# zhengyk19/vit-rpe-rope

Hardware: AMD Instinct MI355X
Metric: train images/sec, CIFAR-10 ViT d=192 L=6 H=6 (higher is better)
Workload: dtype bf16; 1 GPU; CIFAR-10-shaped 32x32 patch4 ViT d=192 L=6 H=6, --pos_encoding rope-axial theta=100, bf16, full train step (fwd+CE+bwd+AdamW), random-init weights; per_gpu_batch=512, global_batch=512, parallelism=dp1, hip_graph=True

## Files before the change

### include/vitpe_debug.h

```cpp
#ifndef VITPE_DEBUG_H
#define VITPE_DEBUG_H
#include "vitpe.h"
#ifdef __cplusplus
extern "C" {
#endif

int vitpe_selftest_mma(int dtype, const void* A, const void* Bt, const void* Brow, float* C_row,
                       float* C_tr, vitpe_stream_t stream);

int vitpe_debug_wgrad_census(int dtype, const vitpe_wgrad_problem* problems, int nprob, unsigned long long* census,
                             vitpe_stream_t stream);
int vitpe_debug_attn_census(const void* xn, const void* wqkv, void* out, const float* cos, const float* sin,
                            int B, unsigned long long* census, vitpe_stream_t stream);
int vitpe_debug_attn32_census(const void* xn, const void* wqkv_wide, void* out, const float* cos, const float* sin,
                              int B, unsigned long long* census, vitpe_stream_t stream);
int vitpe_debug_tail2_census(const void* attn_out, const void* x_in, const void* Wp_packed, const float* bp,
                             const float* gamma, const float* beta, void* x_mid, float* mean2, float* rstd2,
                             void* xn_out, const void* W1_packed, const float* b1, const void* W2_packed,
                             const float* b2, void* gp_out, void* h_out, void* out, float* mean_out, float* rstd_out,
                             int M, int HID, unsigned long long* census, vitpe_stream_t stream);
int vitpe_debug_set_gemm2d_mt(int mt);
int vitpe_debug_set_wgrad_wide(int on);
int vitpe_debug_read_bw(const void* src, long long bytes, int depth, int workgroups, unsigned* sink, vitpe_stream_t stream);
#ifdef __cplusplus
}
#endif
#endif
```

### vit-rpe-rope_amd/csrc/attn.hip

```cpp
#include "attn_common.h"
#include <stdlib.h>
#include <type_traits>

namespace vitpe {

template <typename T, typename C, int KM, int NTH = 384>
VITPE_DEV void stage_tokens(const AttnArgs& a, int b, T* xs, T* hbuf, int hbuf_elems, float* s_tab, float* s_coef,
                            int tid, int nthreads, bool stage_tables) {
  constexpr int CHN = CH<T>::n;
  constexpr int DCH = C::LDX / CHN;
  constexpr int D = C::DD;
  const int N = C::ntok(a);
  const T* xg = reinterpret_cast<const T*>(a.xn) + (size_t)b * N * D;
  const Chunk16 zero = {0u, 0u, 0u, 0u};
  constexpr int TOTAL = C::NP * DCH;
  constexpr int ITERS = (TOTAL + NTH - 1) / NTH;
  Chunk16 v[ITERS];
#pragma unroll
  for (int it = 0; it < ITERS; ++it) {
    const int q = tid + it * nthreads, row = q / DCH, cc = q % DCH;
    v[it] = zero;
    if (q < TOTAL && row < N && cc * CHN < D) v[it] = *reinterpret_cast<const Chunk16*>(xg + (size_t)row * D + cc * CHN);
  }
  if (a.ln_gamma != nullptr) {
// ... 378 lines not shown
VITPE_DEV void stage_rows_plain(const T* src, T* dst, int ld, int N, int tid) {
  constexpr int CHN = CH<T>::n, D = C::DD, CPRW = D / CHN, RPP = NTH / CPRW, ITERS = C::NP / RPP;
  const int cc = tid % CPRW, r0 = tid / CPRW;
  const Chunk16 zero = {0u, 0u, 0u, 0u};
  Chunk16 v[ITERS];
#pragma unroll
  for (int it = 0; it < ITERS; ++it) {
    const int row = r0 + it * RPP;
    v[it] = *reinterpret_cast<const Chunk16*>(src + (size_t)min(row, N - 1) * D + cc * CHN);
    if (row >= N) v[it] = zero;
  }
#pragma unroll
  for (int it = 0; it < ITERS; ++it) *reinterpret_cast<Chunk16*>(dst + (r0 + it * RPP) * ld + cc * CHN) = v[it];
}

template <int HD, int D, int MT, int KM, int NTOK, int IPW, bool LNF, bool MIXED, int PDEG = 7>
__global__ __launch_bounds__(64 * (D / HD) * IPW, 3) void attn_bwd_reg_kernel(AttnArgs a) {
  using T = bf16;
  using C = AttnCfg<T, HD, D, MT, 1, NTOK>;
  constexpr int NT = C::NT, KS = C::KS, HC = C::HC, SC = C::SC, NTH = 64 * C::H;
  static_assert(NT == 2 && HC == 1, "head dimension 32");
  constexpr int CSLD = HD / 2 + 8;
  constexpr int FRAG = 64 * 8;
  constexpr int XS_ELEMS = IPW * C::NP * C::LDX, DOS_ELEMS = IPW * C::H * MT * FRAG;
  __shared__ __attribute__((aligned(16))) T xs_all[XS_ELEMS > DOS_ELEMS ? XS_ELEMS : DOS_ELEMS];
  __shared__ __attribute__((aligned(16))) T qs_all[IPW * C::H * MT * FRAG];
  __shared__ __attribute__((aligned(16))) float s_tab[KM == KM_RELATIVE ? C::H * C::TABLD : 4];
  __shared__ __attribute__((aligned(16))) float s_coef[KM == KM_POLY ? C::PESZ : 4];
  __shared__ __attribute__((aligned(16))) float s_cos[KM == KM_ROPE ? C::NP * CSLD : 4];
  __shared__ __attribute__((aligned(16))) float s_sin[KM == KM_ROPE ? C::NP * CSLD : 4];
  __shared__ __attribute__((aligned(16))) float s_stat[IPW * C::H * 2 * C::NP];
  __shared__ float s_dtab[KM == KM_RELATIVE ? C::H * C::TABLD : 4];
  __shared__ float s_dcoef[C::H * (C::MAXDEG + 1)];
  __shared__ float s_dfreq[2 * C::H * (HD / 2)];

  const int N = C::ntok(a), P = N - 1;
  const int lane = threadIdx.x & 63;
  const int wave_all = __builtin_amdgcn_readfirstlane(threadIdx.x >> 6);
  const int img = wave_all / C::H, h = wave_all % C::H;
  const int b_raw = blockIdx.x * IPW + img;
  const bool live = b_raw < a.B;
  const int b = live ? b_raw : a.B - 1;
  const int tid_img = threadIdx.x % NTH;
  T* const xs = xs_all + img * C::NP * C::LDX;
  T* const qsw = qs_all + wave_all * MT * FRAG + lane * 8;
  T* const dsw = xs_all + wave_all * MT * FRAG + lane * 8;
  float* const lse_w = s_stat + (img * C::H + h) * 2 * C::NP;
  float* const del_w = lse_w + C::NP;
  float* const dtab_i = s_dtab;
  float* const dcoef_i = s_dcoef;
  float* const dfreq_i = s_dfreq;
  const int c = lane & 15, g = lane >> 4;
  const f32x4 z4 = {0.f, 0.f, 0.f, 0.f};
  constexpr bool mixed = (KM == KM_ROPE) && MIXED;

  const T* const Wh = reinterpret_cast<const T*>(a.wqkv) + ((size_t)h * 3 * NT * KS * 64 + lane) * 8;
  auto wload = [&](Frag<T> (&w)[NT][KS], int mat) {
#pragma unroll
    for (int nt = 0; nt < NT; ++nt)
#pragma unroll
      for (int ks = 0; ks < KS; ++ks) w[nt][ks] = ld_frag(Wh + (size_t)((mat * NT + nt) * KS + ks) * 64 * 8);
  };
  Frag<T> w[NT][KS];
  wload(w, 2);
  stage_tokens_fwd<T, C, KM, NTH, LNF>(a, b, xs, s_tab, s_coef, tid_img, false, IPW == 1 || img == 0);
  if (KM == KM_ROPE && !mixed) {
    constexpr int F4 = HD / 8;
    for (int q = threadIdx.x; q < C::NP * F4; q += NTH * IPW) {
      const int f4 = q % F4, row = q / F4;
      f32x4 cv = {1.f, 1.f, 1.f, 1.f}, sv = {0.f, 0.f, 0.f, 0.f};
      if (row >= 1 && row < N) {
        cv = *reinterpret_cast<const f32x4*>(a.cos + (size_t)(row - 1) * (HD / 2) + 4 * f4);
        sv = *reinterpret_cast<const f32x4*>(a.sin + (size_t)(row - 1) * (HD / 2) + 4 * f4);
      }
      *reinterpret_cast<f32x4*>(&s_cos[row * CSLD + 4 * f4]) = cv;
      *reinterpret_cast<f32x4*>(&s_sin[row * CSLD + 4 * f4]) = sv;
    }
  }
  if (KM == KM_RELATIVE)
    for (int q = threadIdx.x; q < C::H * C::TABLD; q += NTH * IPW) s_dtab[q] = 0.f;
  for (int q = threadIdx.x; q < C::H * (C::MAXDEG + 1); q += NTH * IPW) s_dcoef[q] = 0.f;
  for (int q = threadIdx.x; q < 2 * C::H * (HD / 2); q += NTH * IPW) s_dfreq[q] = 0.f;
  __syncthreads();

  const T* const xrow = xs + c * C::LDX + 8 * g;
  const unsigned hoff = mixed ? (unsigned)(h * P * (HD / 2)) : 0u;
  auto cs_vec = [&](int tok, int f, f32x4& cv, f32x4& sv) {
    if (!mixed) {
      cv = *reinterpret_cast<const f32x4*>(&s_cos[tok * CSLD + f]);
      sv = *reinterpret_cast<const f32x4*>(&s_sin[tok * CSLD + f]);
    } else {
      const bool ok = tok >= 1 && tok < N;
      const unsigned o = hoff + (unsigned)((min(max(tok, 1), N - 1) - 1) * (HD / 2) + f);
      const f32x4 cg = *reinterpret_cast<const f32x4*>(a.cos + o), sg = *reinterpret_cast<const f32x4*>(a.sin + o);
      cv = ok ? cg : (f32x4){1.f, 1.f, 1.f, 1.f};
      sv = ok ? sg : z4;
    }
  };
  auto proj_sw = [&](int tt, bool rope, float sc, Frag<T>& dst) {
    Frag<T> xf[KS];
#pragma unroll
    for (int ks = 0; ks < KS; ++ks) xf[ks] = ld_frag(xrow + 16 * tt * C::LDX + 32 * ks);
    __builtin_amdgcn_sched_barrier(0);
    f32x4 acc[NT] = {z4, z4};
#pragma unroll
    for (int ks = 0; ks < KS; ++ks)
#pragma unroll
      for (int nt = 0; nt < NT; ++nt) mma(w[nt][ks], xf[ks], acc[nt]);
    __builtin_amdgcn_sched_barrier(0);
    if (KM == KM_ROPE && rope) {
      f32x4 cv, sv;
      cs_vec(16 * tt + c, 4 * g, cv, sv);
      const f32x4 x1 = acc[0], x2 = acc[1];
      acc[0] = x1 * cv - x2 * sv;
      acc[1] = x1 * sv + x2 * cv;
    }
    dst = acc_to_frag<T>(acc[0] * sc, acc[1] * sc);
    asm volatile("" : "+v"(dst.v));
  };
  Frag<T> e0, e1;
#pragma unroll
  for (int t = 0; t < 8; ++t) {
    e0.v[t] = (bf16)((t < 4 && 4 * g + t == c) ? 1.0f : 0.0f);
    e1.v[t] = (bf16)((t >= 4 && 4 * g + t - 4 == c) ? 1.0f : 0.0f);
  }
  auto transpose_pair = [&](const Frag<T>& fa, const Frag<T>* fb, Frag<T>& d0, Frag<T>& d1) {
    f32x4 a0 = z4, a1 = z4, b0 = z4, b1 = z4;
    mma(fa, e0, a0);
    mma(fa, e1, a1);
    if (fb != nullptr) { mma(*fb, e0, b0); mma(*fb, e1, b1); }
    d0 = acc_to_frag<T>(a0, b0);
    d1 = acc_to_frag<T>(a1, b1);
  };

  const float qsc = a.scale * LOG2E;
  Frag<T> vkf[MT], kf[MT];
#pragma unroll
  for (int tt = 0; tt < MT; ++tt) proj_sw(tt, false, 1.0f, vkf[tt]);
  wload(w, 1);
  __builtin_amdgcn_sched_barrier(0);
#pragma unroll
  for (int tt = 0; tt < MT; ++tt) proj_sw(tt, true, 1.0f, kf[tt]);
  wload(w, 0);
  __builtin_amdgcn_sched_barrier(0);
#pragma unroll
  for (int tt = 0; tt < MT; ++tt) {
    Frag<T> qf;
    proj_sw(tt, true, qsc, qf);
    *reinterpret_cast<bf16x8*>(qsw + tt * FRAG) = qf.v;
  }
  __syncthreads();
  if (!live) return;
  {
    const T* dog = reinterpret_cast<const T*>(a.dout) + (size_t)b * N * D + h * HD;
    Frag<T> df[MT];
#pragma unroll
    for (int tt = 0; tt < MT; ++tt) {
      const int tok = 16 * tt + c;
      bf16x4 lo = {(bf16)0.f, (bf16)0.f, (bf16)0.f, (bf16)0.f}, hi = lo;
      if (tok < N) {
        lo = *reinterpret_cast<const bf16x4*>(dog + (size_t)tok * D + 4 * g);
        hi = *reinterpret_cast<const bf16x4*>(dog + (size_t)tok * D + 16 + 4 * g);
      }
      df[tt].v = __builtin_shufflevector(lo, hi, 0, 1, 2, 3, 4, 5, 6, 7);
    }
#pragma unroll
    for (int tt = 0; tt < MT; ++tt) *reinterpret_cast<bf16x8*>(dsw + tt * FRAG) = df[tt].v;
  }
  auto qf_load = [&](int tt) { Frag<T> f; f.v = *reinterpret_cast<const bf16x8*>(qsw + tt * FRAG); return f; };
  auto dof_load = [&](int tt) { Frag<T> f; f.v = *reinterpret_cast<const bf16x8*>(dsw + tt * FRAG); return f; };
  Frag<T> ktf[NT][SC];
#pragma unroll
  for (int scx = 0; scx < SC; ++scx)
    transpose_pair(kf[2 * scx], (2 * scx + 1 < MT) ? &kf[(2 * scx + 1 < MT) ? 2 * scx + 1 : 0] : nullptr, ktf[0][scx], ktf[1][scx]);

  T* const dqg = reinterpret_cast<T*>(a.out) + (size_t)b * N * 3 * D + h * HD;
  auto store_pair = [&](T* rowp, const f32x4& o0, const f32x4& o1, bool ok) {
    uint32_t lo[2], hi[2];
#pragma unroll
    for (int w2 = 0; w2 < 2; ++w2) {
      bf16x2 pa, pb;
      pa[0] = (bf16)o0[2 * w2]; pa[1] = (bf16)o0[2 * w2 + 1];
      pb[0] = (bf16)o1[2 * w2]; pb[1] = (bf16)o1[2 * w2 + 1];
      const auto r = __builtin_amdgcn_permlane16_swap(__builtin_bit_cast(uint32_t, pa), __builtin_bit_cast(uint32_t, pb), false, false);
      lo[w2] = r[0]; hi[w2] = r[1];
    }
    const int f0 = 16 * (g & 1) + 8 * (g >> 1);
    if (ok) *reinterpret_cast<Chunk16*>(rowp + f0) = (Chunk16){lo[0], lo[1], hi[0], hi[1]};
  };

  float cacc[PDEG + 1];
#pragma unroll
  for (int k = 0; k <= PDEG; ++k) cacc[k] = 0.f;
#pragma unroll
  for (int it = 0; it < MT; ++it) {
    __builtin_amdgcn_sched_barrier(0);
    const int i = 16 * it + c;
    const Frag<T> dof = dof_load(it), qfi = qf_load(it);
    f32x4 s[MT], dp[MT];
    float m = -1e30f;
    typedef __attribute__((ext_vector_type(4))) unsigned u32x4;
    const unsigned xyi = (KM == KM_POLY) ? reinterpret_cast<const unsigned*>(s_coef + C::H * C::PBLD)[i] : 0u;
    const float* const ptab = s_coef + (a.coeff_per_head ? h : 0) * C::PBLD;
    const bool qcls = (it == 0) && (c == 0);
#pragma unroll
    for (int jt = 0; jt < MT; ++jt) {
      s[jt] = z4;
      mma(kf[jt], qfi, s[jt]);
      dp[jt] = z4;
      mma(vkf[jt], dof, dp[jt]);
      const u32x4 xyj = (KM == KM_POLY) ? *reinterpret_cast<const u32x4*>(s_coef + C::H * C::PBLD + 16 * jt + 4 * g) : (u32x4){0u, 0u, 0u, 0u};
#pragma unroll
      for (int r = 0; r < 4; ++r) {
        const int j = 16 * jt + 4 * g + r;
        float v = s[jt][r];
        if (KM == KM_RELATIVE) v += pe_bias2<C, KM>(a, s_tab, s_coef, h, i, j, N);
        if (KM == KM_POLY) {
          const float bv = ptab[__builtin_amdgcn_sad_u8(xyi, xyj[r], 0u)];
          const bool cls = qcls || (jt == 0 && r == 0 && g == 0);
          v += cls ? 0.f : bv;
        }
        if (jt == MT - 1) v = (j < N) ? v : -1e30f;
        s[jt][r] = v;
        m = fmaxf(m, v);
      }
    }
    m = xg_max(m);
    float l = 0.f;
#pragma unroll
    for (int jt = 0; jt < MT; ++jt)
#pragma unroll
      for (int r = 0; r < 4; ++r) { const float p = __builtin_amdgcn_exp2f(s[jt][r] - m); s[jt][r] = p; l += p; }
    l = xg_sum(l);
    const float inv = __builtin_amdgcn_rcpf(l);
    float dl = 0.f;
#pragma unroll
    for (int jt = 0; jt < MT; ++jt)
#pragma unroll
      for (int r = 0; r < 4; ++r) { s[jt][r] *= inv; dl += s[jt][r] * dp[jt][r]; }
    dl = xg_sum(dl);
    if (g == 0) { lse_w[i] = m + __builtin_amdgcn_logf(l); del_w[i] = dl; }
    const bool qvalid = (it < MT - 1) || (i < N);
    float tacc[PDEG + 1];
#pragma unroll
    for (int k = 0; k <= PDEG; ++k) tacc[k] = 0.f;
#pragma unroll
    for (int jt = 0; jt < MT; ++jt) {
      if (KM == KM_POLY) __builtin_amdgcn_sched_barrier(0);
      const u32x4 xyj = (KM == KM_POLY) ? *reinterpret_cast<const u32x4*>(s_coef + C::H * C::PBLD + 16 * jt + 4 * g) : (u32x4){0u, 0u, 0u, 0u};
#pragma unroll
// ... 5 lines not shown
        if (KM == KM_POLY) {
          const float dsk = (jt == 0 && r == 0) ? (g == 0 ? 0.f : ds) : ds;
          const float x = (float)__builtin_amdgcn_sad_u8(xyi, xyj[r], 0u);
          float pw = x;
          tacc[0] += dsk;
#pragma unroll
          for (int k = 1; k <= PDEG; ++k) { tacc[k] = fmaf(dsk, pw, tacc[k]); if (k < PDEG) pw *= x; }
        }
      }
    }
    if (KM == KM_POLY) {
      const float qm = (it == 0 && c == 0) ? 0.f : 1.f;
#pragma unroll
      for (int k = 0; k <= PDEG; ++k) {
        cacc[k] = fmaf(qm, tacc[k], cacc[k]);
        asm volatile("" : "+v"(cacc[k]));
      }
    }
    if (KM == KM_RELATIVE) {
#pragma unroll
      for (int jt = 0; jt < MT; ++jt) {
        float d0, d1;
        tile_diag_sums(dp[jt], lane, d0, d1);
        const int idx0 = 16 * (it - jt) + c + N - 1;
        if (g == 0) {
          if (idx0 >= 0 && idx0 <= 2 * N - 2) atomicAdd(&dtab_i[h * C::TABLD + idx0], d0);
          if (c >= 1 && idx0 - 16 >= 0 && idx0 - 16 <= 2 * N - 2) atomicAdd(&dtab_i[h * C::TABLD + idx0 - 16], d1);
        }
      }
    }
    f32x4 dqa[NT] = {z4, z4};
#pragma unroll
    for (int scx = 0; scx < SC; ++scx) {
      const Frag<T> bs = acc_to_frag<T>(dp[2 * scx], (2 * scx + 1 < MT) ? dp[(2 * scx + 1 < MT) ? 2 * scx + 1 : 0] : z4);
#pragma unroll
      for (int dt = 0; dt < NT; ++dt) mma(ktf[dt][scx], bs, dqa[dt]);
    }
    if (mixed) {
      const bool tok_ok = i >= 1 && i < N;
      f32x4 dph;
#pragma unroll
      for (int r = 0; r < 4; ++r) dph[r] = dqa[1][r] * (float)qfi.v[r] - dqa[0][r] * (float)qfi.v[4 + r];
      mixed_freq_grad_tile(dfreq_i, dph, i, tok_ok, 16 * it, h, C::H, P, a.grid, HD / 2, 4 * g, LN2, lane);
    }
    if (KM == KM_ROPE) {
      f32x4 cv, sv;
      cs_vec(min(i, C::NP - 1), 4 * g, cv, sv);
      const f32x4 d1 = dqa[0], d2 = dqa[1];
      dqa[0] = d1 * cv + d2 * sv;
      dqa[1] = d2 * cv - d1 * sv;
    }
    store_pair(dqg + (size_t)i * 3 * D, dqa[0] * a.scale, dqa[1] * a.scale, qvalid);
  }

  if (KM == KM_POLY) {
#pragma unroll
    for (int k = 0; k <= PDEG; ++k)
      if (k <= a.degree) {
        const float t = wave_sum(cacc[k]);
        if (lane == 0) atomicAdd(&dcoef_i[(a.coeff_per_head ? h : 0) * (C::MAXDEG + 1) + k], t);
      }
  }
  Frag<T> qtf[NT][SC], dotf[NT][SC];
  __builtin_amdgcn_sched_barrier(0);
#pragma unroll
  for (int scx = 0; scx < SC; ++scx) {
    const bool two = 2 * scx + 1 < MT;
    const Frag<T> qa = qf_load(2 * scx), qb = qf_load(two ? 2 * scx + 1 : 0);
    transpose_pair(qa, two ? &qb : nullptr, qtf[0][scx], qtf[1][scx]);
    const Frag<T> da = dof_load(2 * scx), db = dof_load(two ? 2 * scx + 1 : 0);
    transpose_pair(da, two ? &db : nullptr, dotf[0][scx], dotf[1][scx]);
  }
  __builtin_amdgcn_s_waitcnt(0xC07F);

#pragma unroll
  for (int jt = 0; jt < MT; ++jt) {
    __builtin_amdgcn_sched_barrier(0);
    const int j = 16 * jt + c;
    const bool kvalid = (jt < MT - 1) || (j < N);
    const unsigned xyk = (KM == KM_POLY) ? reinterpret_cast<const unsigned*>(s_coef + C::H * C::PBLD)[j] : 0u;
    const float* const ptab2 = s_coef + (a.coeff_per_head ? h : 0) * C::PBLD;
    const bool kcls = (jt == 0) && (c == 0);
    f32x4 p[MT], ds[MT];
#pragma unroll
    for (int it = 0; it < MT; ++it) {
      const Frag<T> dof = dof_load(it), qfi = qf_load(it);
      p[it] = z4;
      mma(qfi, kf[jt], p[it]);
      ds[it] = z4;
      mma(dof, vkf[jt], ds[it]);
      const f32x4 lse = *reinterpret_cast<const f32x4*>(&lse_w[16 * it + 4 * g]);
      const f32x4 dlv = *reinterpret_cast<const f32x4*>(&del_w[16 * it + 4 * g]);
      typedef __attribute__((ext_vector_type(4))) unsigned u32x4;
      const u32x4 xyq = (KM == KM_POLY) ? *reinterpret_cast<const u32x4*>(s_coef + C::H * C::PBLD + 16 * it + 4 * g) : (u32x4){0u, 0u, 0u, 0u};
#pragma unroll
      for (int r = 0; r < 4; ++r) {
        const int i = 16 * it + 4 * g + r;
        float sv = p[it][r];
        if (KM == KM_RELATIVE) sv += pe_bias2<C, KM>(a, s_tab, s_coef, h, i, j, N);
        if (KM == KM_POLY) {
          const float bv = ptab2[__builtin_amdgcn_sad_u8(xyk, xyq[r], 0u)];
          const bool cls = kcls || (it == 0 && r == 0 && g == 0);
          sv += cls ? 0.f : bv;
        }
        const bool valid = kvalid && ((it < MT - 1) || (i < N));
        const float pv = valid ? __builtin_amdgcn_exp2f(sv - lse[r]) : 0.f;
        p[it][r] = pv;
        ds[it][r] = pv * (ds[it][r] - dlv[r]);
      }
    }
    f32x4 dva[NT] = {z4, z4}, dka[NT] = {z4, z4};
#pragma unroll
    for (int scx = 0; scx < SC; ++scx) {
      const bool two = (2 * scx + 1 < MT);
      const Frag<T> bp = acc_to_frag<T>(p[2 * scx], two ? p[two ? 2 * scx + 1 : 0] : z4);
      const Frag<T> bs = acc_to_frag<T>(ds[2 * scx], two ? ds[two ? 2 * scx + 1 : 0] : z4);
#pragma unroll
      for (int dt = 0; dt < NT; ++dt) {
        mma(dotf[dt][scx], bp, dva[dt]);
        mma(qtf[dt][scx], bs, dka[dt]);
      }
    }
    dka[0] *= LN2; dka[1] *= LN2;
    if (mixed) {
      const bool tok_ok = j >= 1 && j < N;
      f32x4 dph;
#pragma unroll
      for (int r = 0; r < 4; ++r) dph[r] = dka[1][r] * (float)kf[jt].v[r] - dka[0][r] * (float)kf[jt].v[4 + r];
      mixed_freq_grad_tile(dfreq_i, dph, j, tok_ok, 16 * jt, h, C::H, P, a.grid, HD / 2, 4 * g, 1.0f, lane);
    }
    if (KM == KM_ROPE) {
      f32x4 cv, sv;
      cs_vec(min(j, C::NP - 1), 4 * g, cv, sv);
      const f32x4 d1 = dka[0], d2 = dka[1];
      dka[0] = d1 * cv + d2 * sv;
      dka[1] = d2 * cv - d1 * sv;
    }
    store_pair(dqg + (size_t)j * 3 * D + D, dka[0], dka[1], kvalid);
    store_pair(dqg + (size_t)j * 3 * D + 2 * D, dva[0], dva[1], kvalid);
  }

  __syncthreads();
  const int nrun = NTH * min(IPW, a.B - (int)blockIdx.x * IPW);
  if (KM == KM_RELATIVE) {
    for (int q = threadIdx.x; q < C::H * (2 * N - 1); q += nrun) {
      const int hh = q / (2 * N - 1), i = q % (2 * N - 1);
      atomicAdd(a.dtable + q, s_dtab[hh * C::TABLD + i]);
    }
  } else if (KM == KM_POLY) {
    const int nh = a.coeff_per_head ? C::H : 1;
    for (int q = threadIdx.x; q < nh * (a.degree + 1); q += nrun) {
      const int hh = q / (a.degree + 1), k = q % (a.degree + 1);
      atomicAdd(a.dcoeff + q, s_dcoef[hh * (C::MAXDEG + 1) + k]);
    }
  } else if (mixed) {
    for (int q = threadIdx.x; q < 2 * C::H * (HD / 2); q += nrun) atomicAdd(a.dfreqs + q, s_dfreq[q]);
  }
}

template <typename T, int HD, int D, int MT, int HPP, int KM, int NTOK>
__global__ __launch_bounds__(384) void attn_bwd_kernel(AttnArgs a) {
  using C = AttnCfg<T, HD, D, MT, HPP, NTOK>;
  __shared__ __attribute__((aligned(16))) T xs[C::NP * C::LDX];
  __shared__ __attribute__((aligned(16))) T hb[4 * HPP * C::HSZ];
  __shared__ __attribute__((aligned(16))) float s_tab[KM == KM_RELATIVE ? C::H * C::TABLD : 4];
  __shared__ __attribute__((aligned(16))) float s_coef[KM == KM_POLY ? C::PESZ : 4];
  __shared__ __attribute__((aligned(16))) float s_stat[HPP * 2 * C::NP];
  __shared__ float s_dtab[KM == KM_RELATIVE ? C::H * C::TABLD : 4];
  __shared__ float s_dcoef[C::H * (C::MAXDEG + 1)];
  __shared__ float s_dfreq[2 * C::H * (HD / 2)];
  constexpr int SLD = HPP * HD + Pad<T>::elems;
  __shared__ __attribute__((aligned(16))) T s_dq[3 * C::NP * SLD];

  const int N = C::ntok(a);
  const int b = blockIdx.x;
  const int lane = threadIdx.x & 63;
  const int wave = __builtin_amdgcn_readfirstlane(threadIdx.x >> 6);
  const int c = lane & 15, g = lane >> 4;
  const int P = N - 1;
  WFrags<T, C> wf;
  {
    const int hh = wave / 3, mat = wave % 3;
    if (hh < HPP && hh < C::H) load_w<T, C>(a, wf, hh, mat, lane);
  }
  stage_tokens<T, C, KM>(a, b, xs, hb, 4 * HPP * C::HSZ, s_tab, s_coef, threadIdx.x, 384, true);
  if (KM == KM_RELATIVE)
    for (int q = threadIdx.x; q < C::H * C::TABLD; q += 384) s_dtab[q] = 0.f;
  for (int q = threadIdx.x; q < C::H * (C::MAXDEG + 1); q += 384) s_dcoef[q] = 0.f;
  for (int q = threadIdx.x; q < 2 * C::H * (HD / 2); q += 384) s_dfreq[q] = 0.f;
  __syncthreads();

  constexpr int CHN = CH<T>::n;
  const T* dog = reinterpret_cast<const T*>(a.dout) + (size_t)b * N * D;
// ... 340 lines not shown
    if (a.ln_gamma != nullptr) hipLaunchKernelGGL((attn_fwd_kernel<T, HD, D, MT, KM, NTOK, IPW, true>), grid, block, 0, s, a);
    else hipLaunchKernelGGL((attn_fwd_kernel<T, HD, D, MT, KM, NTOK, IPW, false>), grid, block, 0, s, a);
  }
  VITPE_CHECK_LAUNCH();
}

template <typename T, int HD, int D, int MT, int HPP, int NTOK>
static int launch_attn2(bool bwd, const AttnArgs& a, hipStream_t s) {
  switch (a.mode) {
    case PE_RELATIVE: return launch_attn3<T, HD, D, MT, HPP, KM_RELATIVE, NTOK>(bwd, a, s);
    case PE_POLY: return launch_attn3<T, HD, D, MT, HPP, KM_POLY, NTOK>(bwd, a, s);
    case PE_ROPE_AXIAL:
    case PE_ROPE_MIXED: return launch_attn3<T, HD, D, MT, HPP, KM_ROPE, NTOK>(bwd, a, s);
    default: return launch_attn3<T, HD, D, MT, HPP, KM_PLAIN, NTOK>(bwd, a, s);
  }
}

template <typename T, int HD, int D, int MT, int HPP>
static int launch_attn(bool bwd, const AttnArgs& a, hipStream_t s) {
  if (a.N == 65) return launch_attn2<T, HD, D, MT, HPP, 65>(bwd, a, s);
  return launch_attn2<T, HD, D, MT, HPP, 0>(bwd, a, s);
}

static int dispatch_attn(bool bwd, int dtype, int D, int HD, const AttnArgs& a, hipStream_t s) {
  const int MT = (a.N + 15) / 16;
  if (HD != 32 || MT != 5) return (int)hipErrorNotSupported;
  if (dtype == 1) {
    if (D == 192) return launch_attn<bf16, 32, 192, 5, 2>(bwd, a, s);
    if (D == 96) return launch_attn<bf16, 32, 96, 5, 2>(bwd, a, s);
  } else if (dtype == 0) {
    if (D == 192) return launch_attn<float, 32, 192, 5, 1>(bwd, a, s);
    if (D == 96) return launch_attn<float, 32, 96, 5, 1>(bwd, a, s);
  }
  return (int)hipErrorNotSupported;
}

extern "C" int vitpe_fused_attention_supported(int dtype, int N, int D, int HD) {
  const int MT = (N + 15) / 16;
  return (dtype == 0 || dtype == 1) && HD == 32 && MT == 5 && (D == 192 || D == 96);
}

static int fused_fwd(int dtype, const void* x, const float* gamma, const float* beta, const float* mean,
                     const float* rstd, void* xn_out, const void* wqkv, void* out, int B, int N, int D, int HD,
                     const PeArgs& pe, hipStream_t stream) {
  VITPE_REQUIRE(x && wqkv && out && B >= 0 && N >= 2);
  VITPE_REQUIRE(pe_ok(pe, N, 0, 0));
  if (B == 0) return 0;
  AttnArgs a = attn_args(pe, B, N, 0, HD);
  a.xn = x; a.wqkv = wqkv; a.out = out;
  a.ln_gamma = gamma; a.ln_beta = beta; a.ln_mean = mean; a.ln_rstd = rstd; a.xn_out = xn_out;
  return dispatch_attn(false, dtype, D, HD, a, stream);
}

static int fused_bwd(int dtype, const void* x, const float* gamma, const float* beta, const float* mean,
                     const float* rstd, const void* wqkv, const void* dout, void* dqkv, int B, int N, int D, int HD,
                     const PeArgs& pe, float* dtable, float* dcoeff, float* dfreqs, hipStream_t stream) {
  VITPE_REQUIRE(x && wqkv && dout && dqkv && B >= 0 && N >= 2);
  VITPE_REQUIRE(pe_ok(pe, N, 0, 0));
  VITPE_REQUIRE(pe_grads_ok(pe.mode, dtable, dcoeff, dfreqs));
  if (B == 0) return 0;
  AttnArgs a = attn_args(pe, B, N, 0, HD);
  a.xn = x; a.wqkv = wqkv; a.out = dqkv; a.dout = dout;
  a.dtable = dtable; a.dcoeff = dcoeff; a.dfreqs = dfreqs;
  a.ln_gamma = gamma; a.ln_beta = beta; a.ln_mean = mean; a.ln_rstd = rstd;
  return dispatch_attn(true, dtype, D, HD, a, stream);
}

extern "C" int vitpe_fused_attention_fwd(int dtype, const void* xn, const void* wqkv, void* out, int B, int N,
                                         int D, int HD, int mode, const float* cos, const float* sin,
                                         const float* table, const float* coeff, int grid, int degree,
                                         int coeff_per_head, hipStream_t stream) {
  return fused_fwd(dtype, xn, nullptr, nullptr, nullptr, nullptr, nullptr, wqkv, out, B, N, D, HD,
                   {mode, cos, sin, table, coeff, grid, degree, coeff_per_head}, stream);
}

extern "C" int vitpe_fused_attention_fwd_ln(int dtype, const void* x, const float* gamma, const float* beta,
                                            const float* mean, const float* rstd, void* xn_out, const void* wqkv,
                                            void* out, int B, int N, int D, int HD, int mode, const float* cos,
                                            const float* sin, const float* table, const float* coeff, int grid,
                                            int degree, int coeff_per_head, hipStream_t stream) {
  VITPE_REQUIRE(gamma && beta && mean && rstd);
  return fused_fwd(dtype, x, gamma, beta, mean, rstd, xn_out, wqkv, out, B, N, D, HD,
                   {mode, cos, sin, table, coeff, grid, degree, coeff_per_head}, stream);
}

extern "C" int vitpe_fused_attention_bwd(int dtype, const void* xn, const void* wqkv, const void* dout,
                                         void* dqkv, int B, int N, int D, int HD, int mode, const float* cos,
                                         const float* sin, const float* table, const float* coeff, int grid,
                                         int degree, int coeff_per_head, float* dtable, float* dcoeff,
                                         float* dfreqs, hipStream_t stream) {
  return fused_bwd(dtype, xn, nullptr, nullptr, nullptr, nullptr, wqkv, dout, dqkv, B, N, D, HD,
                   {mode, cos, sin, table, coeff, grid, degree, coeff_per_head}, dtable, dcoeff, dfreqs, stream);
}

extern "C" int vitpe_fused_attention_bwd_ln(int dtype, const void* x, const float* gamma, const float* beta,
                                            const float* mean, const float* rstd, const void* wqkv, const void* dout,
                                            void* dqkv, int B, int N, int D, int HD, int mode, const float* cos,
                                            const float* sin, const float* table, const float* coeff, int grid,
                                            int degree, int coeff_per_head, float* dtable, float* dcoeff,
                                            float* dfreqs, hipStream_t stream) {
  VITPE_REQUIRE(gamma && beta && mean && rstd);
  return fused_bwd(dtype, x, gamma, beta, mean, rstd, wqkv, dout, dqkv, B, N, D, HD,
                   {mode, cos, sin, table, coeff, grid, degree, coeff_per_head}, dtable, dcoeff, dfreqs, stream);
}

extern "C" int vitpe_debug_attn_census(const void* xn, const void* wqkv, void* out, const float* cos, const float* sin,
                                       int B, unsigned long long* census, hipStream_t stream) {
  VITPE_REQUIRE(xn && wqkv && out && cos && sin && census && B > 0);
  AttnArgs a = attn_args({PE_ROPE_AXIAL, cos, sin, nullptr, nullptr, 8, 0, 0}, B, 65, 0, 32);
  a.xn = xn; a.wqkv = wqkv; a.out = out; a.census = census;
  hipLaunchKernelGGL((attn_fwd_kernel<bf16, 32, 192, 5, KM_ROPE, 65, 2, false, true>), dim3((B + 1) / 2), dim3(768), 0, stream, a);
  VITPE_CHECK_LAUNCH();
}
```

### vit-rpe-rope_amd/csrc/attn_common.h

```cpp
#pragma once
#include "common.h"

namespace vitpe {

struct AttnArgs {
  const void* xn;
  const void* wqkv;
  void* out;
  const void* dout;
  const float* cos;
  const float* sin;
  const float* table;
  const float* coeff;
  float* dtable;
  float* dcoeff;
  float* dfreqs;
  const void* qkv;
  int B, N, H;
  int mode, grid, degree, coeff_per_head;
  float scale;
  const float* ln_gamma;
  const float* ln_beta;
  const float* ln_mean;
  const float* ln_rstd;
  void* xn_out;
  unsigned long long* census;
  void* qkv_out;
  float* tab_slab;
  const unsigned long long* rng;
  unsigned drop_thr;
  float drop_rs;
  int cls_only;
};

struct PeArgs {
  int mode;
  const float *cos, *sin, *table, *coeff;
  int grid, degree, coeff_per_head;
};

inline bool pe_ok(const PeArgs& pe, int N, int H, int hmax) {
  if (pe.mode == PE_ROPE_AXIAL || pe.mode == PE_ROPE_MIXED) {
    if (!pe.cos || !pe.sin || pe.grid * pe.grid != N - 1) return false;
    if (pe.mode == PE_ROPE_MIXED && hmax && H > hmax) return false;
  }
  if (pe.mode == PE_RELATIVE && !pe.table) return false;
  if (pe.mode == PE_POLY && (!pe.coeff || pe.degree < 0 || pe.degree > 7 || pe.grid * pe.grid != N - 1)) return false;
  return pe.mode >= PE_NONE && pe.mode <= PE_ROPE_MIXED;
}

inline bool pe_grads_ok(int mode, const float* dtable, const float* dcoeff, const float* dfreqs) {
  if (mode == PE_RELATIVE) return dtable != nullptr;
  if (mode == PE_POLY) return dcoeff != nullptr;
  if (mode == PE_ROPE_MIXED) return dfreqs != nullptr;
  return true;
}

inline AttnArgs attn_args(const PeArgs& pe, int B, int N, int H, int HD) {
  AttnArgs a{};
  a.cos = pe.cos; a.sin = pe.sin; a.table = pe.table; a.coeff = pe.coeff;
  a.mode = pe.mode; a.grid = pe.grid; a.degree = pe.degree; a.coeff_per_head = pe.coeff_per_head;
  a.B = B; a.N = N; a.H = H;
  a.scale = 1.0f / sqrtf((float)HD);
  return a;
}

constexpr float LOG2E = 1.4426950408889634f;
constexpr float LN2 = 0.6931471805599453f;

enum { KM_PLAIN = 0, KM_RELATIVE = 1, KM_POLY = 2, KM_ROPE = 3, KM_ROPE_TABLES = 4 };

template <typename T, int HD, int D, int MT, int HPP, int NTOK>
struct AttnCfg {
  static constexpr int H = D / HD;
  static constexpr int NT = HD / 16;
  static constexpr int KS = D / 32;
  static constexpr int HC = HD / 32;
  static constexpr int NP = 16 * MT;
  static constexpr int SC = (MT + 1) / 2;
  static constexpr int VR = 32 * SC;
  static constexpr int LDX = D + (sizeof(T) == 2 ? 2 : 1) * Pad<T>::elems;
  static constexpr int LDH = HD + (sizeof(T) == 2 ? 2 : 1) * Pad<T>::elems;
  static constexpr int HSZ = VR * LDH;
  static constexpr int QSZ = NP * LDH;
  static constexpr int TABLD = 2 * NP;
// ... 133 lines not shown
```

### vit-rpe-rope_amd/vitpe/kernels.py

```python
from __future__ import annotations

import ctypes
from typing import Optional, Tuple

import torch

from . import _lib as L
from ._lib import check, dtype_code, lib, ptr, require_device, stream_ptr

SPLITS_TARGET_WGS = 512


def _f32(t, name):
    if t is not None and t.dtype != torch.float32:
        raise L.VitpeError(f"{name} must be float32")


def gemm_nt(a, w, bias=None, epi=L.EPI_BIAS, resid=None, u=None, out=None):
    require_device(a, w, bias, resid, u, out)
    M, K = a.shape
    N = w.shape[0]
    assert w.shape[1] == K and a.dtype == w.dtype
    _f32(bias, "bias")
    c = out if out is not None else torch.empty((M, N), dtype=a.dtype, device=a.device)
# ... 943 lines not shown

def ema_blocks(n: int) -> int:
    return lib().vitpe_ema_blocks(int(n))


def ema_update(p, e, hp, warmup=False):
    require_device(p, e, hp)
    _f32(p, "p"); _f32(e, "e"); _f32(hp, "hp")
    if hp is None or hp.numel() < 16 or e.numel() != p.numel():
        raise L.VitpeError("ema_update: hp must hold 16 floats and e as many elements as p")
    check(lib().vitpe_ema_update(ptr(p), ptr(e), ptr(hp), p.numel(), int(bool(warmup)), stream_ptr()), "vitpe_ema_update")


def ema_swap(p, e, shadow_bf16=None):
    require_device(p, e, shadow_bf16)
    _f32(p, "p"); _f32(e, "e")
    if e.numel() != p.numel() or (shadow_bf16 is not None and (shadow_bf16.dtype != torch.bfloat16 or
                                                               shadow_bf16.numel() != p.numel())):
        raise L.VitpeError("ema_swap: e (fp32) and shadow_bf16 (bf16) must hold as many elements as p")
    check(lib().vitpe_ema_swap(ptr(p), ptr(e), ptr(shadow_bf16), p.numel(), stream_ptr()), "vitpe_ema_swap")


def cast(src, dtype, out=None):
    require_device(src, out)
    _f32(src, "src")
    o = out if out is not None else torch.empty(src.shape, dtype=dtype, device=src.device)
    check(lib().vitpe_cast(dtype_code(dtype), ptr(src), ptr(o), src.numel(), stream_ptr()), "vitpe_cast")
    return o


def transpose_cast(src, dtype, out=None):
    require_device(src, out)
    _f32(src, "src")
    R, C = src.shape
    o = out if out is not None else torch.empty((C, R), dtype=dtype, device=src.device)
    check(lib().vitpe_transpose_cast(dtype_code(dtype), ptr(src), ptr(o), R, C, stream_ptr()), "vitpe_transpose_cast")
    return o


def refresh_shadows(flat, dst_base, desc, ndesc, total_tiles, tile_map=None):
    require_device(flat, dst_base, desc, tile_map)
    assert tile_map is None or (tile_map.dtype == torch.int16 and tile_map.numel() == total_tiles)
    check(lib().vitpe_refresh_shadows(dtype_code(dst_base.dtype), ptr(flat), ptr(dst_base), ptr(desc), ndesc, total_tiles,
                                      ptr(tile_map), stream_ptr()), "vitpe_refresh_shadows")


def selftest_mma(a, bt, brow):
    require_device(a, bt, brow)
    c_row = torch.empty((16, 16), dtype=torch.float32, device=a.device)
    c_tr = torch.empty((16, 16), dtype=torch.float32, device=a.device)
    check(L.debug_lib().vitpe_selftest_mma(dtype_code(a.dtype), ptr(a), ptr(bt), ptr(brow), ptr(c_row), ptr(c_tr),
                                   stream_ptr()), "vitpe_selftest_mma")
    return c_row, c_tr
```

Measured before the change: 381,700 images/sec.

## Skip attention backward tiles whose upstream gradient rows are all zero

The fused attention backward kernel now loads the output-gradient rows first and builds a per-wavefront mask of 16-token tiles that contain any nonzero value. Q projection, the dQ row loop, the transposes and the dK/dV accumulation skip dead tiles and write zeros instead. This targets layers where only some tokens carry gradient, such as the last block when only the CLS token feeds the head. In exchange, every layer pays a ballot plus an earlier dout load, and the kernel gains a separately compiled sparse path. A debug switch can force all tiles live.

Measured after the change: 381,400 images/sec. Within noise of the previous version (-0.1%).

```diff
diff --git a/include/vitpe_debug.h b/include/vitpe_debug.h
--- a/include/vitpe_debug.h
+++ b/include/vitpe_debug.h
@@ -21,6 +21,7 @@
                              int M, int HID, unsigned long long* census, vitpe_stream_t stream);
 int vitpe_debug_set_gemm2d_mt(int mt);
 int vitpe_debug_set_wgrad_wide(int on);
+int vitpe_debug_set_attn_bwd_skip(int on);
 int vitpe_debug_read_bw(const void* src, long long bytes, int depth, int workgroups, unsigned* sink, vitpe_stream_t stream);
 #ifdef __cplusplus
 }
diff --git a/vit-rpe-rope_amd/csrc/attn.hip b/vit-rpe-rope_amd/csrc/attn.hip
--- a/vit-rpe-rope_amd/csrc/attn.hip
+++ b/vit-rpe-rope_amd/csrc/attn.hip
@@ -526,17 +526,28 @@
     e0.v[t] = (bf16)((t < 4 && 4 * g + t == c) ? 1.0f : 0.0f);
     e1.v[t] = (bf16)((t >= 4 && 4 * g + t - 4 == c) ? 1.0f : 0.0f);
   }
-  auto transpose_pair = [&](const Frag<T>& fa, const Frag<T>* fb, Frag<T>& d0, Frag<T>& d1) {
+  auto transpose_pair = [&](const Frag<T>& fa, const Frag<T>& fb, bool two, Frag<T>& d0, Frag<T>& d1) {
     f32x4 a0 = z4, a1 = z4, b0 = z4, b1 = z4;
     mma(fa, e0, a0);
     mma(fa, e1, a1);
-    if (fb != nullptr) { mma(*fb, e0, b0); mma(*fb, e1, b1); }
+    if (two) { mma(fb, e0, b0); mma(fb, e1, b1); }
     d0 = acc_to_frag<T>(a0, b0);
     d1 = acc_to_frag<T>(a1, b1);
   };
 
   const float qsc = a.scale * LOG2E;
   Frag<T> vkf[MT], kf[MT];
+  constexpr unsigned ALL_TILES = (1u << MT) - 1u;
+  typedef __attribute__((ext_vector_type(2))) unsigned u32x2;
+  const T* const dog = reinterpret_cast<const T*>(a.dout) + (size_t)b * N * D + h * HD;
+  u32x2 zlo[MT], zhi[MT];
+#pragma unroll
+  for (int tt = 0; tt < MT; ++tt) {
+    const T* const rowp = dog + (size_t)min(16 * tt + c, N - 1) * D + 4 * g;
+    zlo[tt] = *reinterpret_cast<const u32x2*>(rowp);
+    zhi[tt] = *reinterpret_cast<const u32x2*>(rowp + 16);
+    if (16 * tt + c >= N) { zlo[tt] = (u32x2){0u, 0u}; zhi[tt] = (u32x2){0u, 0u}; }
+  }
 #pragma unroll
   for (int tt = 0; tt < MT; ++tt) proj_sw(tt, false, 1.0f, vkf[tt]);
   wload(w, 1);
@@ -544,37 +555,45 @@
 #pragma unroll
   for (int tt = 0; tt < MT; ++tt) proj_sw(tt, true, 1.0f, kf[tt]);
   wload(w, 0);
+  unsigned tmask = 0u;
+#pragma unroll
+  for (int tt = 0; tt < MT; ++tt) {
+    const unsigned any = (zlo[tt][0] | zlo[tt][1] | zhi[tt][0] | zhi[tt][1]) & 0x7fff7fffu;
+    if (__builtin_amdgcn_ballot_w64(any != 0u) != 0ull) tmask |= 1u << tt;
+  }
+  tmask = __builtin_amdgcn_readfirstlane(a.all_live ? ALL_TILES : tmask);
   __builtin_amdgcn_sched_barrier(0);
-#pragma unroll
-  for (int tt = 0; tt < MT; ++tt) {
-    Frag<T> qf;
-    proj_sw(tt, true, qsc, qf);
-    *reinterpret_cast<bf16x8*>(qsw + tt * FRAG) = qf.v;
+  if (tmask == ALL_TILES) {
+#pragma unroll
+    for (int tt = 0; tt < MT; ++tt) {
+      Frag<T> qf;
+      proj_sw(tt, true, qsc, qf);
+      *reinterpret_cast<bf16x8*>(qsw + tt * FRAG) = qf.v;
+    }
+  } else {
+#pragma unroll
+    for (int tt = 0; tt < MT; ++tt) {
+      Frag<T> qf;
+#pragma unroll
+      for (int t = 0; t < 8; ++t) qf.v[t] = (bf16)0.f;
+      if ((tmask >> tt) & 1u) proj_sw(tt, true, qsc, qf);
+      *reinterpret_cast<bf16x8*>(qsw + tt * FRAG) = qf.v;
+    }
   }
   __syncthreads();
   if (!live) return;
   {
-    const T* dog = reinterpret_cast<const T*>(a.dout) + (size_t)b * N * D + h * HD;
-    Frag<T> df[MT];
-#pragma unroll
-    for (int tt = 0; tt < MT; ++tt) {
-      const int tok = 16 * tt + c;
-      bf16x4 lo = {(bf16)0.f, (bf16)0.f, (bf16)0.f, (bf16)0.f}, hi = lo;
-      if (tok < N) {
-        lo = *reinterpret_cast<const bf16x4*>(dog + (size_t)tok * D + 4 * g);
-        hi = *reinterpret_cast<const bf16x4*>(dog + (size_t)tok * D + 16 + 4 * g);
-      }
-      df[tt].v = __builtin_shufflevector(lo, hi, 0, 1, 2, 3, 4, 5, 6, 7);
-    }
-#pragma unroll
-    for (int tt = 0; tt < MT; ++tt) *reinterpret_cast<bf16x8*>(dsw + tt * FRAG) = df[tt].v;
+    typedef __attribute__((ext_vector_type(4))) unsigned u32x4;
+#pragma unroll
+    for (int tt = 0; tt < MT; ++tt)
+      *reinterpret_cast<u32x4*>(dsw + tt * FRAG) = (u32x4){zlo[tt][0], zlo[tt][1], zhi[tt][0], zhi[tt][1]};
   }
   auto qf_load = [&](int tt) { Frag<T> f; f.v = *reinterpret_cast<const bf16x8*>(qsw + tt * FRAG); return f; };
   auto dof_load = [&](int tt) { Frag<T> f; f.v = *reinterpret_cast<const bf16x8*>(dsw + tt * FRAG); return f; };
   Frag<T> ktf[NT][SC];
 #pragma unroll
   for (int scx = 0; scx < SC; ++scx)
-    transpose_pair(kf[2 * scx], (2 * scx + 1 < MT) ? &kf[(2 * scx + 1 < MT) ? 2 * scx + 1 : 0] : nullptr, ktf[0][scx], ktf[1][scx]);
+    transpose_pair(kf[2 * scx], kf[(2 * scx + 1 < MT) ? 2 * scx + 1 : 0], 2 * scx + 1 < MT, ktf[0][scx], ktf[1][scx]);
 
   T* const dqg = reinterpret_cast<T*>(a.out) + (size_t)b * N * 3 * D + h * HD;
   auto store_pair = [&](T* rowp, const f32x4& o0, const f32x4& o1, bool ok) {
@@ -590,6 +609,11 @@
     const int f0 = 16 * (g & 1) + 8 * (g >> 1);
     if (ok) *reinterpret_cast<Chunk16*>(rowp + f0) = (Chunk16){lo[0], lo[1], hi[0], hi[1]};
   };
+  auto store_zero = [&](T* rowp, bool ok) {
+    if (ok) *reinterpret_cast<Chunk16*>(rowp + 16 * (g & 1) + 8 * (g >> 1)) = (Chunk16){0u, 0u, 0u, 0u};
+  };
+
+  auto on = [&](int t) { return ((tmask >> t) & 1u) != 0u; };
 
   float cacc[PDEG + 1];
 #pragma unroll
@@ -598,6 +622,10 @@
   for (int it = 0; it < MT; ++it) {
     __builtin_amdgcn_sched_barrier(0);
     const int i = 16 * it + c;
+    if (!on(it)) {
+      store_zero(dqg + (size_t)i * 3 * D, (it < MT - 1) || (i < N));
+      continue;
+    }
     const Frag<T> dof = dof_load(it), qfi = qf_load(it);
     f32x4 s[MT], dp[MT];
     float m = -1e30f;
@@ -710,7 +738,7 @@
     store_pair(dqg + (size_t)i * 3 * D, dqa[0] * a.scale, dqa[1] * a.scale, qvalid);
   }
 
-  if (KM == KM_POLY) {
+  if (KM == KM_POLY && tmask != 0u) {
 #pragma unroll
     for (int k = 0; k <= PDEG; ++k)
       if (k <= a.degree) {
@@ -718,29 +746,40 @@
         if (lane == 0) atomicAdd(&dcoef_i[(a.coeff_per_head ? h : 0) * (C::MAXDEG + 1) + k], t);
       }
   }
+  auto pair_live = [&](int scx) { return on(2 * scx) || (2 * scx + 1 < MT && on(2 * scx + 1)); };
   Frag<T> qtf[NT][SC], dotf[NT][SC];
   __builtin_amdgcn_sched_barrier(0);
 #pragma unroll
   for (int scx = 0; scx < SC; ++scx) {
     const bool two = 2 * scx + 1 < MT;
+    if (!pair_live(scx)) continue;
     const Frag<T> qa = qf_load(2 * scx), qb = qf_load(two ? 2 * scx + 1 : 0);
-    transpose_pair(qa, two ? &qb : nullptr, qtf[0][scx], qtf[1][scx]);
+    transpose_pair(qa, qb, two, qtf[0][scx], qtf[1][scx]);
     const Frag<T> da = dof_load(2 * scx), db = dof_load(two ? 2 * scx + 1 : 0);
-    transpose_pair(da, two ? &db : nullptr, dotf[0][scx], dotf[1][scx]);
+    transpose_pair(da, db, two, dotf[0][scx], dotf[1][scx]);
   }
   __builtin_amdgcn_s_waitcnt(0xC07F);
 
+  auto step2 = [&](const bool SPARSE) __attribute__((always_inline)) {
+  auto on = [&](int t) { return !SPARSE || ((tmask >> t) & 1u) != 0u; };
+  auto pair_on = [&](int scx) { return on(2 * scx) || (2 * scx + 1 < MT && on(2 * scx + 1)); };
 #pragma unroll
   for (int jt = 0; jt < MT; ++jt) {
     __builtin_amdgcn_sched_barrier(0);
     const int j = 16 * jt + c;
     const bool kvalid = (jt < MT - 1) || (j < N);
+    if (SPARSE && tmask == 0u) {
+      store_zero(dqg + (size_t)j * 3 * D + D, kvalid);
+      store_zero(dqg + (size_t)j * 3 * D + 2 * D, kvalid);
+      continue;
+    }
     const unsigned xyk = (KM == KM_POLY) ? reinterpret_cast<const unsigned*>(s_coef + C::H * C::PBLD)[j] : 0u;
     const float* const ptab2 = s_coef + (a.coeff_per_head ? h : 0) * C::PBLD;
     const bool kcls = (jt == 0) && (c == 0);
     f32x4 p[MT], ds[MT];
 #pragma unroll
     for (int it = 0; it < MT; ++it) {
+      if (!on(it)) { p[it] = z4; ds[it] = z4; continue; }
       const Frag<T> dof = dof_load(it), qfi = qf_load(it);
       p[it] = z4;
       mma(qfi, kf[jt], p[it]);
@@ -770,6 +809,7 @@
 #pragma unroll
     for (int scx = 0; scx < SC; ++scx) {
       const bool two = (2 * scx + 1 < MT);
+      if (!pair_on(scx)) continue;
       const Frag<T> bp = acc_to_frag<T>(p[2 * scx], two ? p[two ? 2 * scx + 1 : 0] : z4);
       const Frag<T> bs = acc_to_frag<T>(ds[2 * scx], two ? ds[two ? 2 * scx + 1 : 0] : z4);
 #pragma unroll
@@ -796,6 +836,9 @@
     store_pair(dqg + (size_t)j * 3 * D + D, dka[0], dka[1], kvalid);
     store_pair(dqg + (size_t)j * 3 * D + 2 * D, dva[0], dva[1], kvalid);
   }
+  };
+  if (tmask == ALL_TILES) step2(false);
+  else step2(true);
 
   __syncthreads();
   const int nrun = NTH * min(IPW, a.B - (int)blockIdx.x * IPW);
@@ -1242,6 +1285,9 @@
   return dispatch_attn(false, dtype, D, HD, a, stream);
 }
 
+static bool g_bwd_skip = true;
+extern "C" int vitpe_debug_set_attn_bwd_skip(int on) { g_bwd_skip = on != 0; return 0; }
+
 static int fused_bwd(int dtype, const void* x, const float* gamma, const float* beta, const float* mean,
                      const float* rstd, const void* wqkv, const void* dout, void* dqkv, int B, int N, int D, int HD,
                      const PeArgs& pe, float* dtable, float* dcoeff, float* dfreqs, hipStream_t stream) {
@@ -1253,6 +1299,7 @@
   a.xn = x; a.wqkv = wqkv; a.out = dqkv; a.dout = dout;
   a.dtable = dtable; a.dcoeff = dcoeff; a.dfreqs = dfreqs;
   a.ln_gamma = gamma; a.ln_beta = beta; a.ln_mean = mean; a.ln_rstd = rstd;
+  a.all_live = g_bwd_skip ? 0 : 1;
   return dispatch_attn(true, dtype, D, HD, a, stream);
 }
 
diff --git a/vit-rpe-rope_amd/csrc/attn_common.h b/vit-rpe-rope_amd/csrc/attn_common.h
--- a/vit-rpe-rope_amd/csrc/attn_common.h
+++ b/vit-rpe-rope_amd/csrc/attn_common.h
@@ -31,6 +31,7 @@
   unsigned drop_thr;
   float drop_rs;
   int cls_only;
+  int all_live;
 };
 
 struct PeArgs {
diff --git a/vit-rpe-rope_amd/vitpe/kernels.py b/vit-rpe-rope_amd/vitpe/kernels.py
--- a/vit-rpe-rope_amd/vitpe/kernels.py
+++ b/vit-rpe-rope_amd/vitpe/kernels.py
@@ -1019,3 +1019,7 @@
     check(L.debug_lib().vitpe_selftest_mma(dtype_code(a.dtype), ptr(a), ptr(bt), ptr(brow), ptr(c_row), ptr(c_tr),
                                    stream_ptr()), "vitpe_selftest_mma")
     return c_row, c_tr
+
+
+def debug_set_attn_bwd_skip(on: bool):
+    check(L.debug_lib().vitpe_debug_set_attn_bwd_skip(1 if on else 0), "vitpe_debug_set_attn_bwd_skip")
```

## Skip non-CLS query backward work when attention output gradient is CLS-only

Applied to the files above, without the earlier changes.

Adds a runtime check in the fused attention backward kernel that detects when the incoming gradient is zero for all non-CLS tokens, as happens in the last ViT layer. In that case it recomputes only the first query tile, runs a reduced backward core specialised for one query tile, and writes zeros for the other dQ rows. This removes most of the query-side MMA work for that layer. The cost is an extra gradient-sparsity probe in every layer and larger code and register pressure from two instantiations of the core.

After: 385,000 images/sec before, 387,300 images/sec after (median of 6 runs). No clear change (+0.6%).

```diff
diff --git a/include/vitpe_debug.h b/include/vitpe_debug.h
--- a/include/vitpe_debug.h
+++ b/include/vitpe_debug.h
@@ -21,6 +21,7 @@
                              int M, int HID, unsigned long long* census, vitpe_stream_t stream);
 int vitpe_debug_set_gemm2d_mt(int mt);
 int vitpe_debug_set_wgrad_wide(int on);
+int vitpe_debug_set_attn_bwd_cls(int on);
 int vitpe_debug_read_bw(const void* src, long long bytes, int depth, int workgroups, unsigned* sink, vitpe_stream_t stream);
 #ifdef __cplusplus
 }
diff --git a/vit-rpe-rope_amd/csrc/attn.hip b/vit-rpe-rope_amd/csrc/attn.hip
--- a/vit-rpe-rope_amd/csrc/attn.hip
+++ b/vit-rpe-rope_amd/csrc/attn.hip
@@ -454,6 +454,7 @@
   float* const dfreq_i = s_dfreq;
   const int c = lane & 15, g = lane >> 4;
   const f32x4 z4 = {0.f, 0.f, 0.f, 0.f};
+  constexpr bool FAST = (KM == KM_PLAIN || KM == KM_ROPE);
   constexpr bool mixed = (KM == KM_ROPE) && MIXED;
 
   const T* const Wh = reinterpret_cast<const T*>(a.wqkv) + ((size_t)h * 3 * NT * KS * 64 + lane) * 8;
@@ -544,20 +545,43 @@
 #pragma unroll
   for (int tt = 0; tt < MT; ++tt) proj_sw(tt, true, 1.0f, kf[tt]);
   wload(w, 0);
+  bool only_cls = false;
+  if (FAST && a.bwd_cls) {
+    const T* const dz = reinterpret_cast<const T*>(a.dout) + (size_t)b * N * D + h * HD + 8 * (lane & 3);
+    unsigned nz = 0u;
+    if (lane < 4) {
+      const Chunk16 v = *reinterpret_cast<const Chunk16*>(dz + D);
+      nz = v[0] | v[1] | v[2] | v[3];
+    }
+    if (__builtin_amdgcn_ballot_w64((nz & 0x7fff7fffu) != 0u) == 0ull) {
+#pragma unroll
+      for (int k = 0; k < MT; ++k)
+        if (16 * k + 1 < N) {
+          const Chunk16 v = *reinterpret_cast<const Chunk16*>(dz + (size_t)min(16 * k + 1 + (lane >> 2), N - 1) * D);
+          nz |= v[0] | v[1] | v[2] | v[3];
+        }
+      only_cls = __builtin_amdgcn_ballot_w64((nz & 0x7fff7fffu) != 0u) == 0ull;
+    }
+  }
   __builtin_amdgcn_sched_barrier(0);
 #pragma unroll
   for (int tt = 0; tt < MT; ++tt) {
-    Frag<T> qf;
-    proj_sw(tt, true, qsc, qf);
-    *reinterpret_cast<bf16x8*>(qsw + tt * FRAG) = qf.v;
+    if (tt == 0 || !only_cls) {
+      Frag<T> qf;
+      proj_sw(tt, true, qsc, qf);
+      *reinterpret_cast<bf16x8*>(qsw + tt * FRAG) = qf.v;
+    }
   }
   __syncthreads();
   if (!live) return;
+  auto core = [&](auto cls_tag, const int lane, const int c, const int g, T* const qsw, T* const dsw) {
+  constexpr bool CLS = decltype(cls_tag)::value;
+  constexpr int MTQ = CLS ? 1 : MT, SCQ = CLS ? 1 : SC;
   {
     const T* dog = reinterpret_cast<const T*>(a.dout) + (size_t)b * N * D + h * HD;
-    Frag<T> df[MT];
-#pragma unroll
-    for (int tt = 0; tt < MT; ++tt) {
+    Frag<T> df[MTQ];
+#pragma unroll
+    for (int tt = 0; tt < MTQ; ++tt) {
       const int tok = 16 * tt + c;
       bf16x4 lo = {(bf16)0.f, (bf16)0.f, (bf16)0.f, (bf16)0.f}, hi = lo;
       if (tok < N) {
@@ -567,7 +591,7 @@
       df[tt].v = __builtin_shufflevector(lo, hi, 0, 1, 2, 3, 4, 5, 6, 7);
     }
 #pragma unroll
-    for (int tt = 0; tt < MT; ++tt) *reinterpret_cast<bf16x8*>(dsw + tt * FRAG) = df[tt].v;
+    for (int tt = 0; tt < MTQ; ++tt) *reinterpret_cast<bf16x8*>(dsw + tt * FRAG) = df[tt].v;
   }
   auto qf_load = [&](int tt) { Frag<T> f; f.v = *reinterpret_cast<const bf16x8*>(qsw + tt * FRAG); return f; };
   auto dof_load = [&](int tt) { Frag<T> f; f.v = *reinterpret_cast<const bf16x8*>(dsw + tt * FRAG); return f; };
@@ -595,7 +619,7 @@
 #pragma unroll
   for (int k = 0; k <= PDEG; ++k) cacc[k] = 0.f;
 #pragma unroll
-  for (int it = 0; it < MT; ++it) {
+  for (int it = 0; it < MTQ; ++it) {
     __builtin_amdgcn_sched_barrier(0);
     const int i = 16 * it + c;
     const Frag<T> dof = dof_load(it), qfi = qf_load(it);
@@ -709,6 +733,14 @@
     }
     store_pair(dqg + (size_t)i * 3 * D, dqa[0] * a.scale, dqa[1] * a.scale, qvalid);
   }
+  if constexpr (CLS) {
+    const Chunk16 zero = {0u, 0u, 0u, 0u};
+#pragma unroll
+    for (int k = 1; k < MT; ++k) {
+      const int row = 16 * k + (lane >> 2);
+      if (row < N) *reinterpret_cast<Chunk16*>(dqg + (size_t)row * 3 * D + 8 * (lane & 3)) = zero;
+    }
+  }
 
   if (KM == KM_POLY) {
 #pragma unroll
@@ -718,11 +750,11 @@
         if (lane == 0) atomicAdd(&dcoef_i[(a.coeff_per_head ? h : 0) * (C::MAXDEG + 1) + k], t);
       }
   }
-  Frag<T> qtf[NT][SC], dotf[NT][SC];
+  Frag<T> qtf[NT][SCQ], dotf[NT][SCQ];
   __builtin_amdgcn_sched_barrier(0);
 #pragma unroll
-  for (int scx = 0; scx < SC; ++scx) {
-    const bool two = 2 * scx + 1 < MT;
+  for (int scx = 0; scx < SCQ; ++scx) {
+    const bool two = 2 * scx + 1 < MTQ;
     const Frag<T> qa = qf_load(2 * scx), qb = qf_load(two ? 2 * scx + 1 : 0);
     transpose_pair(qa, two ? &qb : nullptr, qtf[0][scx], qtf[1][scx]);
     const Frag<T> da = dof_load(2 * scx), db = dof_load(two ? 2 * scx + 1 : 0);
@@ -730,17 +762,19 @@
   }
   __builtin_amdgcn_s_waitcnt(0xC07F);
 
+  int c2 = c;
+  asm volatile("" : "+v"(c2));
 #pragma unroll
   for (int jt = 0; jt < MT; ++jt) {
     __builtin_amdgcn_sched_barrier(0);
-    const int j = 16 * jt + c;
+    const int j = 16 * jt + c2;
     const bool kvalid = (jt < MT - 1) || (j < N);
     const unsigned xyk = (KM == KM_POLY) ? reinterpret_cast<const unsigned*>(s_coef + C::H * C::PBLD)[j] : 0u;
     const float* const ptab2 = s_coef + (a.coeff_per_head ? h : 0) * C::PBLD;
     const bool kcls = (jt == 0) && (c == 0);
-    f32x4 p[MT], ds[MT];
-#pragma unroll
-    for (int it = 0; it < MT; ++it) {
+    f32x4 p[MTQ], ds[MTQ];
+#pragma unroll
+    for (int it = 0; it < MTQ; ++it) {
       const Frag<T> dof = dof_load(it), qfi = qf_load(it);
       p[it] = z4;
       mma(qfi, kf[jt], p[it]);
@@ -768,8 +802,8 @@
     }
     f32x4 dva[NT] = {z4, z4}, dka[NT] = {z4, z4};
 #pragma unroll
-    for (int scx = 0; scx < SC; ++scx) {
-      const bool two = (2 * scx + 1 < MT);
+    for (int scx = 0; scx < SCQ; ++scx) {
+      const bool two = (2 * scx + 1 < MTQ);
       const Frag<T> bp = acc_to_frag<T>(p[2 * scx], two ? p[two ? 2 * scx + 1 : 0] : z4);
       const Frag<T> bs = acc_to_frag<T>(ds[2 * scx], two ? ds[two ? 2 * scx + 1 : 0] : z4);
 #pragma unroll
@@ -795,6 +829,22 @@
     }
     store_pair(dqg + (size_t)j * 3 * D + D, dka[0], dka[1], kvalid);
     store_pair(dqg + (size_t)j * 3 * D + 2 * D, dva[0], dva[1], kvalid);
+  }
+  };
+  if (only_cls) {
+    int lane_f = lane;
+    asm volatile("" : "+v"(lane_f));
+#pragma unroll
+    for (int tt = 0; tt < MT; ++tt) { asm volatile("" : "+v"(kf[tt].v)); asm volatile("" : "+v"(vkf[tt].v)); }
+#pragma unroll
+    for (int t = 0; t < 8; ++t) {
+      e0.v[t] = (bf16)((t < 4 && 4 * (lane_f >> 4) + t == (lane_f & 15)) ? 1.0f : 0.0f);
+      e1.v[t] = (bf16)((t >= 4 && 4 * (lane_f >> 4) + t - 4 == (lane_f & 15)) ? 1.0f : 0.0f);
+    }
+    const int off_f = wave_all * MT * FRAG + lane_f * 8;
+    core(std::true_type{}, lane_f, lane_f & 15, lane_f >> 4, qs_all + off_f, xs_all + off_f);
+  } else {
+    core(std::false_type{}, lane, c, g, qsw, dsw);
   }
 
   __syncthreads();
@@ -1242,6 +1292,9 @@
   return dispatch_attn(false, dtype, D, HD, a, stream);
 }
 
+static bool g_bwd_cls = true;
+extern "C" int vitpe_debug_set_attn_bwd_cls(int on) { g_bwd_cls = on != 0; return 0; }
+
 static int fused_bwd(int dtype, const void* x, const float* gamma, const float* beta, const float* mean,
                      const float* rstd, const void* wqkv, const void* dout, void* dqkv, int B, int N, int D, int HD,
                      const PeArgs& pe, float* dtable, float* dcoeff, float* dfreqs, hipStream_t stream) {
@@ -1253,6 +1306,7 @@
   a.xn = x; a.wqkv = wqkv; a.out = dqkv; a.dout = dout;
   a.dtable = dtable; a.dcoeff = dcoeff; a.dfreqs = dfreqs;
   a.ln_gamma = gamma; a.ln_beta = beta; a.ln_mean = mean; a.ln_rstd = rstd;
+  a.bwd_cls = g_bwd_cls ? 1 : 0;
   return dispatch_attn(true, dtype, D, HD, a, stream);
 }
 
diff --git a/vit-rpe-rope_amd/csrc/attn_common.h b/vit-rpe-rope_amd/csrc/attn_common.h
--- a/vit-rpe-rope_amd/csrc/attn_common.h
+++ b/vit-rpe-rope_amd/csrc/attn_common.h
@@ -31,6 +31,7 @@
   unsigned drop_thr;
   float drop_rs;
   int cls_only;
+  int bwd_cls;
 };
 
 struct PeArgs {
diff --git a/vit-rpe-rope_amd/vitpe/kernels.py b/vit-rpe-rope_amd/vitpe/kernels.py
--- a/vit-rpe-rope_amd/vitpe/kernels.py
+++ b/vit-rpe-rope_amd/vitpe/kernels.py
@@ -1019,3 +1019,7 @@
     check(L.debug_lib().vitpe_selftest_mma(dtype_code(a.dtype), ptr(a), ptr(bt), ptr(brow), ptr(c_row), ptr(c_tr),
                                    stream_ptr()), "vitpe_selftest_mma")
     return c_row, c_tr
+
+
+def set_attn_bwd_cls(on: bool):
+    check(L.debug_lib().vitpe_debug_set_attn_bwd_cls(1 if on else 0), "vitpe_debug_set_attn_bwd_cls")
```
